# dbdexter-dev/meteor_demod

Measured on AMD Instinct MI355X. Metric: IQ Msamples/s demodulated (whole node), higher is better.
Workload: dtype f32

## Files before the change

meteor_demod_amd/csrc/demod_device.h:

```cpp
#ifndef MDEMOD_DEVICE_H
#define MDEMOD_DEVICE_H

#include <hip/hip_runtime.h>
#include <stdint.h>

#include "pll_flags.h"

#pragma clang fp contract(off)

#define MD_TWO_PI_D 6.283185307179586476925286766559
#define MD_HALF_PI_D 1.5707963267948966192313216916398
#define MD_TWO_PI_F 6.28318548202514648437500f
#define MD_PI_F     3.14159274101257324218750f

struct cf32 { float re, im; };

__device__ __forceinline__ bool md_any(bool p) { return __builtin_amdgcn_ballot_w64(p) != 0ull; }
__device__ __forceinline__ bool md_all(bool p) { return __builtin_amdgcn_ballot_w64(!p) == 0ull; }

template <typename T>
__device__ __forceinline__ T md_lane_select(uint64_t mask, T a, T b)
{
	static_assert(sizeof(T) == 4, "one 32-bit register");
	T r;
// ... 82 lines not shown
{
	return md_fast_sin<CHECKED>((float)((double)fx + MD_HALF_PI_D));
}

__device__ __forceinline__ double
md_sqrt_sumsq(double s)
{
	const double y = __builtin_amdgcn_rsq(s);
	double g = s * y;
	double h = 0.5 * y;
	const double r = __builtin_fma(-h, g, 0.5);
	g = __builtin_fma(g, r, g);
	h = __builtin_fma(h, r, h);
	double d = __builtin_fma(-g, g, s);
	g = __builtin_fma(d, h, g);
	d = __builtin_fma(-g, g, s);
	g = __builtin_fma(d, h, g);
	return __builtin_amdgcn_class(s, 0x260) ? s : g;
}

__device__ __forceinline__ float
md_cabsf_exact(float re, float im)
{
	const double s = (double)re * (double)re + (double)im * (double)im;
	return (float)md_sqrt_sumsq(s);
}

__device__ __forceinline__ float
md_cabsf(float re, float im)
{
	return md_cabsf_exact(re, im);
}

__device__ __forceinline__ float
md_cabsf_short(float re, float im, uint32_t *fallbacks = nullptr)
{
	const double s = (double)re * (double)re + (double)im * (double)im;
	const double y = __builtin_amdgcn_rsq(s);
	const double g = s * y, h = 0.5 * y;
	const double d = __builtin_fma(-g, g, s);
	const double g1 = __builtin_fma(d, h, g);
	const uint64_t gb = __builtin_bit_cast(uint64_t, g1), sb = __builtin_bit_cast(uint64_t, s);
	const uint32_t drop = (uint32_t)gb & 0x1FFFFFFFu;
	const bool near = (uint32_t)(drop - (0x10000000u - 0x1000u)) < 0x2000u;
	const bool odd = (uint32_t)((uint32_t)(sb >> 32) - ((1023u - 200u) << 20)) >= (400u << 20);
	float r = (float)g1;
	if (__builtin_expect(near || odd, 0)) {
		r = (float)md_sqrt_sumsq(s);
		if (fallbacks) *fallbacks += 1;
	}
	return r;
}

__device__ __forceinline__ cf32
md_agc_apply(cf32 x, float gain, float &bias_re, float &bias_im)
{
	const float keep = 1.0f - 0.001f;
	bias_re = bias_re * keep + 0.001f * x.re;
	bias_im = bias_im * keep + 0.001f * x.im;
	x.re = x.re - bias_re;
	x.im = x.im - bias_im;
	x.re = x.re * gain;
	x.im = x.im * gain;
	return x;
}

template <bool SHORT = false>
__device__ __forceinline__ void
md_agc_gain(cf32 scaled, float &gain)
{
	const float mag = SHORT ? md_cabsf_short(scaled.re, scaled.im) : md_cabsf(scaled.re, scaled.im);
	gain = gain + 0.0001f * (190.0f - mag);
	gain = (0.0f > gain) ? 0.0f : gain;
}

template <bool SHORT = false>
__device__ __forceinline__ cf32
md_agc(cf32 x, float &gain, float &bias_re, float &bias_im)
{
	x = md_agc_apply(x, gain, bias_re, bias_im);
	md_agc_gain<SHORT>(x, gain);
	return x;
}

#define MD_TWO_PI_LO (-0x1.777a5cp-23f)

template <bool F32 = false>
__device__ __forceinline__ void
md_nco_advance(float &phase, float freq)
{
	phase = phase + freq;
	if (F32) {
		const float w = (phase - MD_TWO_PI_F) - MD_TWO_PI_LO;
		phase = (phase >= MD_TWO_PI_F) ? w : phase;
	} else if (phase >= MD_TWO_PI_F)
		phase = (float)((double)phase - MD_TWO_PI_D);
}

#define MD_FOUR_PI_F 12.56637096405029296875f
__device__ __forceinline__ float
md_wrap_2pi(float xf)
{
	const bool wraps = !(fabsf(xf) < MD_TWO_PI_F);
	const float once = (xf < 0.0f) ? (xf + MD_TWO_PI_F) + MD_TWO_PI_LO : (xf - MD_TWO_PI_F) - MD_TWO_PI_LO;
	float r = wraps ? once : xf;
	const bool far = !(fabsf(xf) < MD_FOUR_PI_F);
	if (__builtin_expect(md_any(far), 0)) {
		if (far) r = (float)fmod((double)xf, MD_TWO_PI_D);
	}
	return r;
}

__device__ __forceinline__ float
md_tanh_lut(const float *lut, float v)
{
	const float c = __builtin_amdgcn_fmed3f(v, -16.0f, 15.0f);
	return lut[(int)c + 16];
}

__device__ __forceinline__ float
md_tanh_lut_uniform(const float *lut, float v)
{
	float t = (v >= 15.0f) ? 1.0f : -1.0f;
	if (__builtin_expect(md_any(v > -16.0f && v < 15.0f), 0)) t = md_tanh_lut(lut, v);
	return t;
}

__device__ __forceinline__ void
md_tanh_lut_uniform2(const float *lut, float a, float b, float &ta, float &tb)
{
	ta = (a >= 15.0f) ? 1.0f : -1.0f;
	tb = (b >= 15.0f) ? 1.0f : -1.0f;
	if (__builtin_expect(md_any((a > -16.0f && a < 15.0f) || (b > -16.0f && b < 15.0f)), 0)) {
		ta = md_tanh_lut(lut, a);
		tb = md_tanh_lut(lut, b);
	}
}

struct PllState {
	float phase, freq, err;
	int   locked, locked_once, updown;
};

template <bool UNIFORM = false>
__device__ __forceinline__ int
md_pll_update(PllState &p, const float *lut, float alpha, float beta, float fmax,
              float i, float q, int &just_locked_first)
{
	const float e = UNIFORM ? md_tanh_lut_uniform(lut, i) * q - md_tanh_lut_uniform(lut, q) * i
	                        : md_tanh_lut(lut, i) * q - md_tanh_lut(lut, q) * i;

	const float ph = p.phase + alpha * e;
	p.phase = md_wrap_2pi(ph);
	p.freq = p.freq + beta * e;

	const float decayed = p.err * (1.0f - 0.001f);
	p.err = (float)((double)decayed + fabs((double)e) * (double)0.001f);

	const bool lock_now = (p.err < 85.0f) && !p.locked;
	const bool unlock_now = (p.err > 105.0f) && p.locked;
	just_locked_first = (lock_now && !p.locked_once) ? 1 : 0;
	p.locked = lock_now ? 1 : (unlock_now ? 0 : p.locked);
	p.locked_once = lock_now ? 1 : p.locked_once;
	const int changed = (lock_now || unlock_now) ? 1 : 0;
// ... 7 lines not shown
	p.freq = (-fmax > p.freq) ? -fmax : p.freq;
	return changed;
}

struct PllWord { float phase, freq, err; };
template <bool UNIFORM = false, bool EARLY_OUT = false>
__device__ __forceinline__ uint32_t
md_pll_update_packed(PllWord &p, uint32_t &fl, const float *lut, float alpha, float beta, float fmax, float i, float q, uint32_t &first)
{
	float ti, tq;
	if (UNIFORM) md_tanh_lut_uniform2(lut, i, q, ti, tq);
	else { ti = md_tanh_lut(lut, i); tq = md_tanh_lut(lut, q); }
	const float e = ti * q - tq * i;

	const float ph = p.phase + alpha * e;
	p.phase = md_wrap_2pi(ph);
	p.freq = p.freq + beta * e;

	const float decayed = p.err * (1.0f - 0.001f);
	p.err = (float)((double)decayed + fabs((double)e) * (double)0.001f);

	if constexpr (EARLY_OUT) {
		const uint64_t m_below = __builtin_amdgcn_ballot_w64(p.err < 85.0f), m_above = __builtin_amdgcn_ballot_w64(p.err > 105.0f);
		const uint64_t m_locked = __builtin_amdgcn_ballot_w64((fl & 1u) != 0);
		const uint64_t m_lock_event = (m_below & ~m_locked) | (m_above & m_locked);
		const float swept = (float)((double)p.freq + ((fl & 4u) ? 0.000001 : -0.000001));
		p.freq = md_lane_select(m_locked ^ m_lock_event, swept, p.freq);
		const uint64_t m_turn = __builtin_amdgcn_ballot_w64(fabsf(p.freq) >= fmax);
		first = 0;
		uint32_t changed = 0;
		if (__builtin_expect((m_lock_event | m_turn) != 0ull, 0)) {
			const PllFlagStep s = pll_flags_step(fl, md_lane_bit(m_below), md_lane_bit(m_above),
			                                     p.freq >= fmax ? PLL_FREQ_HIGH : (p.freq <= -fmax ? PLL_FREQ_LOW : PLL_FREQ_INSIDE));
			fl = s.fl; first = s.first; changed = s.changed;
		}
		p.freq = md_clamp_sym(p.freq, fmax);
		return changed;
	}

	const uint32_t below = (p.err < 85.0f) ? 1u : 0u, above = (p.err > 105.0f) ? 1u : 0u;
	const uint32_t lock_now = below & (fl ^ 1u);
	const uint32_t unlock_now = above & fl;
	const uint32_t lock2 = lock_now + lock_now;
	first = lock2 ^ (lock2 & fl);
	fl = fl | lock_now | lock2;
	fl = fl ^ (fl & unlock_now);

	if (!(fl & 1u)) p.freq = (float)((double)p.freq + ((fl & 4u) ? 0.000001 : -0.000001));
	fl = (p.freq >= fmax) ? (fl & ~4u) : ((p.freq <= -fmax) ? (fl | 4u) : fl);
	p.freq = md_clamp_sym(p.freq, fmax);
	return lock_now | unlock_now;
}

__device__ __forceinline__ void
md_timing_update(float &t_phase, float &t_freq, float &t_prev,
                 float alpha, float beta, float center, float maxdev, float q)
{
	const float sp = (t_prev < 0.0f) ? -1.0f : 1.0f;
	const float sq = (q < 0.0f) ? -1.0f : 1.0f;
	const float e = sp * q - sq * t_prev;
	t_prev = q;

	float fd = t_freq - center;
	t_phase = (float)((double)t_phase - (MD_TWO_PI_D + (double)(alpha * e)));
	fd = fd - beta * e;
	fd = md_clamp_sym(fd, maxdev);
	t_freq = center + fd;
}

__device__ __forceinline__ int
md_quantise(float v)
{
	const float h = md_clamp_sym(v * 0.5f, 127.0f);
	return (int)h;
}

#endif
```

meteor_demod_amd/csrc/demod_kernel_gat.hip:

```cpp
#include "rotwin_body.h"
#include "hip_host.h"

namespace {

typedef float gpair_t __attribute__((ext_vector_type(2)));
typedef float gquad_t __attribute__((ext_vector_type(4)));
typedef __attribute__((address_space(3))) const gquad_t lds_gquad;
typedef __attribute__((address_space(3))) const float lds_gfloat;

template <int FMT> struct GFmt;
template <> struct GFmt<16> {
	enum { G = 4 };
	__device__ static __forceinline__ gpair_t get(const uint4 &q, int k) { const uint32_t w = (&q.x)[k]; return gpair_t{ (float)(int)(int16_t)(w & 0xFFFFu), (float)((int)w >> 16) }; }
	__device__ static __forceinline__ gpair_t one(uint32_t w) { return gpair_t{ (float)(int)(int16_t)(w & 0xFFFFu), (float)((int)w >> 16) }; }
};
template <> struct GFmt<8> {
	enum { G = 8 };
	__device__ static __forceinline__ gpair_t get(const uint4 &q, int k) { const uint32_t w = (&q.x)[k >> 1] >> (16 * (k & 1)); return gpair_t{ (float)((int)(w & 0xFFu) - 128), (float)((int)((w >> 8) & 0xFFu) - 128) }; }
	__device__ static __forceinline__ gpair_t one(uint16_t w) { return gpair_t{ (float)((int)(w & 0xFFu) - 128), (float)((int)(w >> 8) - 128) }; }
};
template <> struct GFmt<32> {
	enum { G = 2 };
	__device__ static __forceinline__ gpair_t get(const uint4 &q, int k) { return gpair_t{ __uint_as_float((&q.x)[2 * k]), __uint_as_float((&q.x)[2 * k + 1]) }; }
	__device__ static __forceinline__ gpair_t one(float2 w) { return gpair_t{ w.x, w.y }; }
};

template <int KT, int FMT>
struct WinG {
	static constexpr int G = GFmt<FMT>::G, kTaps = KT, kBack = KT - 1, AMAX = G - 1, NS = KT + AMAX, NW = 4 * ((NS + 3) / 4), SLIDE = 4, MAXSL = 1, DEPTH = 1,
	                     BLOCK = MDEMOD_RW_BLOCK, ROTN = 1, RING = 32, REGSLOTS = 0;
	static constexpr bool GATHER = true, SCALAR_SLIDE = false, VCONST = false;
	static constexpr bool LOCK_EARLY_OUT = true;
	static_assert(NS % G == 0 && NS / G <= 36, "whole 16-byte loads, and few enough of them to stay in registers");
	typedef typename RFmt<FMT>::sample_t sample_t;
	__device__ __forceinline__ void setup(uint32_t) {}
	__device__ static __forceinline__ void put_history(const float2 *, bool, int) {}
	__device__ static __forceinline__ void put_init(const RGran<FMT> (&)[1], int) {}
	__device__ static __forceinline__ void put(const RGran<FMT> (&)[1], int) {}
	__device__ static __forceinline__ void fir(uint32_t, int, int, const DemodConsts &, int, float &, float &) {}

	__device__ static __forceinline__ void
	fir_gather(uint32_t ctab_addr, const sample_t *src, const float2 *hist, int v, int n, int bank, const DemodConsts &C, float &re, float &im)
	{
		const int oldest = v - kBack - (KT - 1);
		const int d = oldest & (G - 1);
		const int start = oldest - d;
		const int o = AMAX - d;
		const uint32_t row = ctab_addr + 4u * (uint32_t)(__mul24(bank * 4 + (o & 3), C.ctab_row_stride) + (o & ~3));
		gpair_t acc = { 0.0f, 0.0f };
		if (__builtin_expect(md_all(start >= 0 && start + NS <= n), 1)) {
			uint4 raw[NS / G];
#pragma unroll
			for (int g = 0; g < NS / G; g++) __builtin_memcpy(&raw[g], src + start + G * g, 16);
#pragma unroll
			for (int s4 = 0; s4 < NS / 4; s4++) {
				gquad_t c = { 0.0f, 0.0f, 0.0f, 0.0f };
				c = *(lds_gquad *)(row + 16u * (uint32_t)s4);
				const float cf[4] = { c.x, c.y, c.z, c.w };
#pragma unroll
				for (int k = 0; k < 4; k++) {
					const int slot = 4 * s4 + k;
					const gpair_t smp = GFmt<FMT>::get(raw[slot / G], slot % G);
					const gpair_t p = smp * cf[k];
					acc = acc + p;
				}
			}
			if constexpr (NS % 4 != 0) {
#pragma unroll
				for (int slot = NS / 4 * 4; slot < NS; slot++) {
					const float cf = *(lds_gfloat *)(row + 4u * (uint32_t)slot);
					const gpair_t p = GFmt<FMT>::get(raw[slot / G], slot % G) * cf;
					acc = acc + p;
				}
			}
		} else {
#pragma unroll 1
			for (int k = 0; k < KT; k++) {
				const int idx = oldest + k;
				gpair_t smp;
				if (idx < 0) { const float2 h = hist[kBack + idx]; smp.x = h.x; smp.y = h.y; }
				else smp = GFmt<FMT>::one(src[idx]);
				const float cf = *(lds_gfloat *)(row + 4u * (uint32_t)(d + k));
				const gpair_t p = smp * cf;
				acc = acc + p;
			}
// ... 44 lines not shown
```

meteor_demod_amd/csrc/demod_kernel_rot.hip:

```cpp
#include "rotwin_body.h"
#include "rot_fir_bounds.h"
#include "hip_host.h"
#ifdef ROTWIN_ASM_HEADER
#include ROTWIN_ASM_HEADER
#else
#include "rotwin_asm.h"
#endif

namespace {

static_assert(ROTWIN_NCH * 8 == 80 && ROTWIN_SLIDE == 8, "window = ten chunks of eight, a slide brings one");


__device__ __forceinline__ void
rot_fir(uint32_t row_addr, int rot, int flags, float &re, float &im)
{
	int tmp;
#if ROTWIN_PK == 1 || ROTWIN_PK == 3
	typedef float pair_t __attribute__((ext_vector_type(2)));
	pair_t acc, p0, p1;
	asm volatile(ROTWIN_FIR_ASM
	             : [acc] "=&v"(acc), [p0] "=&v"(p0), [p1] "=&v"(p1), [tmp] "=&s"(tmp)
	             : [addr] "v"(row_addr), [rot] "s"(rot), [flags] "s"(flags)
	             : "vcc", "scc", ROTWIN_COEF_CLOBBERS);
// ... 13 lines not shown
{
	int tmp;
	asm volatile(ROTWIN_PUT_S16_ASM
	             : [tmp] "=&s"(tmp), [rot] "+s"(q), [base] "+s"(base)
	             : [g0] "v"(a.w[0]), [g1] "v"(a.w[1]), [g2] "v"(a.w[2]), [g3] "v"(a.w[3]),
	               [g4] "v"(b.w[0]), [g5] "v"(b.w[1]), [g6] "v"(b.w[2]), [g7] "v"(b.w[3])
	             : "vcc", "scc", "v255", "memory");
}
template <> __device__ __forceinline__ void
rot_put<8>(const RGran<8> &a, const RGran<8> &b, int &q, int &base)
{
	const uint32_t g0 = a.w[0] ^ 0x80808080u, g1 = a.w[1] ^ 0x80808080u, g2 = b.w[0] ^ 0x80808080u, g3 = b.w[1] ^ 0x80808080u;
	int tmp;
	asm volatile(ROTWIN_PUT_U8_ASM
	             : [tmp] "=&s"(tmp), [rot] "+s"(q), [base] "+s"(base)
	             : [g0] "v"(g0), [g1] "v"(g1), [g2] "v"(g2), [g3] "v"(g3)
	             : "vcc", "scc", "v255", "memory");
}
__device__ __forceinline__ void
rot_put_floats(const uint32_t (&f)[16], int &q, int &base)
{
	int tmp;
	asm volatile(ROTWIN_PUT_F32_ASM
	             : [tmp] "=&s"(tmp), [rot] "+s"(q), [base] "+s"(base)
	             : [f0] "v"(f[0]), [f1] "v"(f[1]), [f2] "v"(f[2]), [f3] "v"(f[3]), [f4] "v"(f[4]), [f5] "v"(f[5]), [f6] "v"(f[6]), [f7] "v"(f[7]),
	               [f8] "v"(f[8]), [f9] "v"(f[9]), [f10] "v"(f[10]), [f11] "v"(f[11]), [f12] "v"(f[12]), [f13] "v"(f[13]), [f14] "v"(f[14]), [f15] "v"(f[15])
	             : "vcc", "scc", "v255", "memory");
}
__device__ __forceinline__ void
rot_put_floats(const uint32_t (&f)[16], int q)
{
	int base = 0;
	rot_put_floats(f, q, base);
}
template <> __device__ __forceinline__ void
rot_put<32>(const RGran<32> &a, const RGran<32> &b, int &q, int &base)
{
	uint32_t f[16];
#pragma unroll
	for (int i = 0; i < 8; i++) { f[i] = a.w[i]; f[8 + i] = b.w[i]; }
	rot_put_floats(f, q, base);
}

template <int FMT, int COMPACT = 0, int BLK = MDEMOD_RW_BLOCK, int VC = 0, int RSL = 0>
struct WinF {
	static constexpr int kTaps = 65, kBack = 64, NW = 80, SLIDE = 8, AMAX = NW - kTaps, MAXSL = 1, DEPTH = 1, BLOCK = BLK, ROTN = NW / SLIDE, RING = 32;
	static constexpr bool GATHER = false;
	static constexpr bool SCALAR_SLIDE = true;
	static constexpr bool VCONST = VC != 0;
	static_assert(SLIDE == ROTWIN_SLIDE && ROTN == ROTWIN_NCH, "the slide's assembly counts for itself");
	__device__ __forceinline__ void setup(uint32_t) {}
	static constexpr int REGSLOTS = RSL;
	static constexpr bool LOCK_EARLY_OUT = true;
	__device__ static __forceinline__ void put_history(const float2 *hist, bool valid, int q)
	{
		const uint4 *h4 = reinterpret_cast<const uint4 *>(hist);
		uint32_t f[16];
#pragma unroll
		for (int i = 0; i < 4; i++) {
			uint4 h = h4[i];
			if (!valid) h = make_uint4(0, 0, 0, 0);
			f[4 * i] = h.x; f[4 * i + 1] = h.y; f[4 * i + 2] = h.z; f[4 * i + 3] = h.w;
		}
		rot_put_floats(f, q);
	}
	__device__ static __forceinline__ void put(const RGran<FMT> (&g)[2], int q) { int base = 0; rot_put<FMT>(g[0], g[1], q, base); }
	__device__ static __forceinline__ void put_init(const RGran<FMT> (&g)[2], int q) { put(g, q); }
	__device__ static __forceinline__ void slide(const RGran<FMT> (&g)[2], int &rot, int &base) { rot_put<FMT>(g[0], g[1], rot, base); }
	__device__ static __forceinline__ void fir(uint32_t ctab_addr, int a, int bank, const DemodConsts &C, int rot, float &re, float &im)
	{
		const int o = AMAX - a;
		uint32_t row_addr;
		if (COMPACT) row_addr = rot_mad24((uint32_t)(bank * 4 + (o & 3)), 4u * (uint32_t)C.ctab_row_stride, ctab_addr + 4u * (uint32_t)(o & ~3));
		else row_addr = rot_mad24(rot_mad24((uint32_t)a, (uint32_t)C.interp, (uint32_t)bank), 4u * (uint32_t)C.ctab_row_stride, ctab_addr);
		static_assert(AMAX == 15, "two bits of a / 4");
		const uint64_t ex = __builtin_amdgcn_ballot_w64(true);
		const RotFirQ q = rot_fir_q(ex, __builtin_amdgcn_ballot_w64(a >= 4), __builtin_amdgcn_ballot_w64(a >= 8), __builtin_amdgcn_ballot_w64(a >= 12));
		int q_hi = q.q_hi;
		asm("" : "+s"(q_hi));
		const int flags = rot_fir_flags(q.q_lo, q_hi);
#ifdef ROT_EXP_NOSKIP
		int f0 = __builtin_amdgcn_readfirstlane(flags);
		asm volatile("s_and_b32 %0, %0, 0" : "+s"(f0) : : "scc");
		rot_fir(row_addr, rot, f0, re, im);
#else
		rot_fir(row_addr, rot, flags, re, im);
#endif
	}
};

typedef float pair_t2 __attribute__((ext_vector_type(2)));

template <int NA>
__device__ __forceinline__ void
rot_fir_acc(uint32_t addr, int rot, int last, pair_t2 &acc)
{
	int tmp;
	if constexpr (NA == 10)
		asm volatile(ROTWIN_FIR_ACC_ASM
		             : [acc] "+v"(acc), [tmp] "=&s"(tmp)
		             : [addr] "v"(addr), [rot] "s"(rot), [last] "s"(last)
		             : "vcc", "scc", ROTWIN_COEF_CLOBBERS, ROTWIN_ACC_CLOBBERS);
	else if constexpr (NA == 2)
		asm volatile(ROTWIN_FIR_ACC2_ASM
		             : [acc] "+v"(acc), [tmp] "=&s"(tmp)
		             : [addr] "v"(addr), [rot] "s"(rot), [last] "s"(last)
		             : "vcc", "scc", ROTWIN_COEF_CLOBBERS, ROTWIN_ACC_CLOBBERS);
	else
		asm volatile(ROTWIN_FIR_ACC5_ASM
		             : [acc] "+v"(acc), [tmp] "=&s"(tmp)
		             : [addr] "v"(addr), [rot] "s"(rot), [last] "s"(last)
		             : "vcc", "scc", ROTWIN_COEF_CLOBBERS, ROTWIN_ACC_CLOBBERS);
}
#define ROT_F16_OPERANDS \
	[f0] "v"(f[0]), [f1] "v"(f[1]), [f2] "v"(f[2]), [f3] "v"(f[3]), [f4] "v"(f[4]), [f5] "v"(f[5]), [f6] "v"(f[6]), [f7] "v"(f[7]), \
	[f8] "v"(f[8]), [f9] "v"(f[9]), [f10] "v"(f[10]), [f11] "v"(f[11]), [f12] "v"(f[12]), [f13] "v"(f[13]), [f14] "v"(f[14]), [f15] "v"(f[15])
template <int NA>
__device__ __forceinline__ void
rot_migrate(const uint32_t (&f)[16], int q)
{
	int tmp;
	if constexpr (NA == 10)
		asm volatile(ROTWIN_MIGRATE_ASM : [tmp] "=&s"(tmp) : ROT_F16_OPERANDS, [rot] "s"(q) : "vcc", "scc", "v255", ROTWIN_ACC_CLOBBERS, "memory");
	else if constexpr (NA == 2)
		asm volatile(ROTWIN_MIGRATE2_ASM : [tmp] "=&s"(tmp) : ROT_F16_OPERANDS, [rot] "s"(q) : "vcc", "scc", "v255", ROTWIN_ACC_CLOBBERS, "memory");
	else
		asm volatile(ROTWIN_MIGRATE5_ASM : [tmp] "=&s"(tmp) : ROT_F16_OPERANDS, [rot] "s"(q) : "vcc", "scc", "v255", ROTWIN_ACC_CLOBBERS, "memory");
}
template <int NA>
__device__ __forceinline__ void
rot_put_acc(const uint32_t (&f)[16], int q)
{
	int tmp;
	if constexpr (NA == 10)
		asm volatile(ROTWIN_PUT_ACC_ASM : [tmp] "=&s"(tmp) : ROT_F16_OPERANDS, [rot] "s"(q) : "vcc", "scc", ROTWIN_ACC_CLOBBERS, "memory");
	else if constexpr (NA == 2)
		asm volatile(ROTWIN_PUT_ACC2_ASM : [tmp] "=&s"(tmp) : ROT_F16_OPERANDS, [rot] "s"(q) : "vcc", "scc", ROTWIN_ACC_CLOBBERS, "memory");
	else
		asm volatile(ROTWIN_PUT_ACC5_ASM : [tmp] "=&s"(tmp) : ROT_F16_OPERANDS, [rot] "s"(q) : "vcc", "scc", ROTWIN_ACC_CLOBBERS, "memory");
}

template <int BLK, int NA, int MSL>
struct WinH {
	static constexpr int NR = 10, SLIDE = 8, NW = SLIDE * (NR + NA), kTaps = NA == 10 ? 129 : 65, kBack = kTaps - 1, AMAX = NW - kTaps, MAXSL = MSL, DEPTH = MSL,
	                     BLOCK = BLK, ROTN = NR, RING = 32, REGSLOTS = 0;
	static constexpr bool GATHER = false, SCALAR_SLIDE = false, VCONST = false;
	static constexpr bool LOCK_EARLY_OUT = true;
	static_assert((NA == 10 || NA == 2 || NA == 5) && AMAX == (NA == 5 ? 55 : 31) && kBack % SLIDE == 0, "wide (160 slots, 129 taps), mid (96 slots, 65 taps) or far (120 slots, 65 taps)");
	__device__ __forceinline__ void setup(uint32_t) {}
	__device__ static __forceinline__ void place(const uint32_t (&f)[16], int c)
	{
		if (c < NR) rot_put_floats(f, c);
		else rot_put_acc<NA>(f, c - NR);
	}
	__device__ static __forceinline__ void put_history(const float2 *hist, bool valid, int c)
	{
		const uint4 *h4 = reinterpret_cast<const uint4 *>(hist);
		uint32_t f[16];
#pragma unroll
		for (int i = 0; i < 4; i++) {
			uint4 h = h4[i];
			if (!valid) h = make_uint4(0, 0, 0, 0);
			f[4 * i] = h.x; f[4 * i + 1] = h.y; f[4 * i + 2] = h.z; f[4 * i + 3] = h.w;
		}
		place(f, c);
	}
	__device__ static __forceinline__ void put_init(const RGran<32> (&g)[2], int c)
	{
		uint32_t f[16];
#pragma unroll
		for (int i = 0; i < 8; i++) { f[i] = g[0].w[i]; f[8 + i] = g[1].w[i]; }
		place(f, c);
	}
	__device__ static __forceinline__ void put(const RGran<32> (&g)[2], int q)
	{
		uint32_t f[16];
#pragma unroll
		for (int i = 0; i < 8; i++) { f[i] = g[0].w[i]; f[8 + i] = g[1].w[i]; }
		rot_migrate<NA>(f, q);
	}
	__device__ static __forceinline__ void fir(uint32_t ctab_addr, int a, int bank, const DemodConsts &C, int rot, float &re, float &im)
	{
		const int o = AMAX - a;
		const uint32_t row = ctab_addr + 4u * (uint32_t)(__mul24(bank * 4 + (o & 3), C.ctab_row_stride) + (o & ~3));
		const int flags = (md_all(a >= 8) ? 3 : 0) | ((NA != 10 && md_all(a <= 7)) ? 16 : 0);
		rot_fir(row, rot, __builtin_amdgcn_readfirstlane(flags), re, im);
		if (NA == 10 || md_any(a >= 16)) {
			int last;
			if (NA == 10) last = 6 + (md_any(a >= 8) ? 1 : 0) + (md_any(a >= 16) ? 1 : 0) + (md_any(a >= 24) ? 1 : 0);
			else {
				last = md_any(a >= 24) ? 1 : 0;
				if (NA == 5) last += (md_any(a >= 32) ? 1 : 0) + (md_any(a >= 40) ? 1 : 0) + (md_any(a >= 48) ? 1 : 0);
			}
			pair_t2 acc = { re, im };
			rot_fir_acc<NA>(row + 4u * 80u, NA == 10 ? rot : (NA == 2 ? (rot & 1) : (rot >= 5 ? rot - 5 : rot)), __builtin_amdgcn_readfirstlane(last), acc);
			re = acc.x; im = acc.y;
		}
	}
};

// ... 69 lines not shown
```

meteor_demod_amd/csrc/demod_kernel_rotp.hip:

```cpp
#include "rotwin_body.h"
#include "hip_host.h"
#ifdef ROTPK_ASM_HEADER
#include ROTPK_ASM_HEADER
#else
#include "rotpk_asm.h"
#endif

namespace {

typedef float pair_t __attribute__((ext_vector_type(2)));

template <int GEO> struct GeoP;
#ifndef ROTP_WIDE_DEPTH
#define ROTP_WIDE_DEPTH 1
#endif
#ifndef ROTP_MID_DEPTH
#define ROTP_MID_DEPTH 1
#endif
#ifndef ROTP_FAR_DEPTH
#define ROTP_FAR_DEPTH 2
#endif
template <> struct GeoP<0> { static constexpr int kTaps = 129, NW = MDEMOD_RW_WIDE_NW, MAXSL = 1, DEPTH = ROTP_WIDE_DEPTH, BLOCK = MDEMOD_RW_WIDE_BLOCK; };
template <> struct GeoP<1> { static constexpr int kTaps = 65, NW = MDEMOD_RW_MID_NW, MAXSL = 1, DEPTH = ROTP_MID_DEPTH, BLOCK = MDEMOD_RW_BLOCK; };
#ifndef ROTP_FAR_MAXSL
// ... 6 lines not shown
#if ROTPK_FORM == 0
#define ROTP_FIR_CALL(TEXT, CLOB)                                                                                             \
	float ar = 0.0f, ai = 0.0f;                                                                                               \
	asm volatile(TEXT : [ar] "+v"(ar), [ai] "+v"(ai), [addr] "+v"(addr), [cnt] "+s"(cnt), [tmp] "=&s"(tmp)                    \
	             : [entry] "s"(entry), [sub] "s"(sub) : "vcc", "scc", CLOB);                                                \
	re = ar; im = ai;
#else
#define ROTP_FIR_CALL(TEXT, CLOB)                                                                                             \
	pair_t acc = { 0.0f, 0.0f };                                                                                              \
	asm volatile(TEXT : [acc] "+v"(acc), [addr] "+v"(addr), [cnt] "+s"(cnt), [tmp] "=&s"(tmp)                                 \
	             : [entry] "s"(entry), [sub] "s"(sub) : "vcc", "scc", CLOB);                                                \
	re = acc.x; im = acc.y;
#endif
#define ROTP_ASM(GEO, NAME, FMT)                                                                                              \
	template <> struct AsmP<GEO, FMT> {                                                                                       \
		__device__ static __forceinline__ void fir(uint32_t addr, int entry, int sub, int cnt, float &re, float &im)          \
		{                                                                                                                     \
			int tmp;                                                                                                          \
			ROTP_FIR_CALL(ROTPK_##NAME##_##FMT##_FIR_ASM, ROTPK_##NAME##_##FMT##_CLOBBERS)                                     \
		}                                                                                                                     \
		__device__ static __forceinline__ void put(const uint32_t (&g)[FMT == 16 ? 16 : 8], int q);                           \
	};
ROTP_ASM(0, WIDE, 16) ROTP_ASM(0, WIDE, 8) ROTP_ASM(1, MID, 16) ROTP_ASM(1, MID, 8) ROTP_ASM(2, FAR, 16) ROTP_ASM(2, FAR, 8)

#define ROTP_PUT16(GEO, NAME)                                                                                                 \
	__device__ __forceinline__ void AsmP<GEO, 16>::put(const uint32_t (&g)[16], int q)                                        \
	{                                                                                                                         \
		int tmp;                                                                                                              \
		asm volatile(ROTPK_##NAME##_16_PUT_ASM                                                                                \
		             : [tmp] "=&s"(tmp)                                                                                       \
		             : [g0] "v"(g[0]), [g1] "v"(g[1]), [g2] "v"(g[2]), [g3] "v"(g[3]), [g4] "v"(g[4]), [g5] "v"(g[5]), [g6] "v"(g[6]),  \
		               [g7] "v"(g[7]), [g8] "v"(g[8]), [g9] "v"(g[9]), [g10] "v"(g[10]), [g11] "v"(g[11]), [g12] "v"(g[12]),  \
		               [g13] "v"(g[13]), [g14] "v"(g[14]), [g15] "v"(g[15]), [rot] "s"(q)                                     \
		             : "vcc", "scc", "v255", "memory");                                                                       \
	}
#define ROTP_PUT8(GEO, NAME)                                                                                                  \
	__device__ __forceinline__ void AsmP<GEO, 8>::put(const uint32_t (&g)[8], int q)                                          \
	{                                                                                                                         \
		int tmp;                                                                                                              \
		asm volatile(ROTPK_##NAME##_8_PUT_ASM                                                                                 \
		             : [tmp] "=&s"(tmp)                                                                                       \
		             : [g0] "v"(g[0]), [g1] "v"(g[1]), [g2] "v"(g[2]), [g3] "v"(g[3]), [g4] "v"(g[4]), [g5] "v"(g[5]), [g6] "v"(g[6]),  \
		               [g7] "v"(g[7]), [rot] "s"(q)                                                                           \
		             : "vcc", "scc", "v255", "memory");                                                                       \
	}
ROTP_PUT16(0, WIDE) ROTP_PUT16(1, MID) ROTP_PUT16(2, FAR) ROTP_PUT8(0, WIDE) ROTP_PUT8(1, MID) ROTP_PUT8(2, FAR)

template <int GEO, int FMT>
struct WinP {
	static constexpr int kTaps = GeoP<GEO>::kTaps, kBack = kTaps - 1, NW = GeoP<GEO>::NW, SLIDE = 16, AMAX = NW - kTaps,
	                     MAXSL = GeoP<GEO>::MAXSL, DEPTH = GeoP<GEO>::DEPTH, BLOCK = GeoP<GEO>::BLOCK, NCH = NW / SLIDE, GD = FMT == 16 ? 16 : 8, REGSLOTS = 0, ROTN = NCH, RING = 32;
	static constexpr bool GATHER = false, SCALAR_SLIDE = false, VCONST = false;
	static constexpr bool LOCK_EARLY_OUT = true;
	__device__ __forceinline__ void setup(uint32_t) {}
	static_assert(kBack % SLIDE == 0 && NW % SLIDE == 0, "history and window are whole chunks");

	__device__ static __forceinline__ void put_history(const float2 *hist, bool valid, int q)
	{
		uint32_t g[GD];
#pragma unroll
		for (int k = 0; k < 16; k++) {
			float2 h = hist[k];
			if (!valid) h = make_float2(0.0f, 0.0f);
			if (FMT == 16) {
				g[k] = ((uint32_t)(int)h.x & 0xFFFFu) | ((uint32_t)(int)h.y << 16);
			} else {
				const uint32_t s = (uint32_t)(((int)h.x + 128) & 0xFF) | ((uint32_t)(((int)h.y + 128) & 0xFF) << 8);
				if (k & 1) g[k / 2] |= s << 16; else g[k / 2] = s;
			}
		}
		AsmP<GEO, FMT>::put(g, q);
	}
	__device__ static __forceinline__ void put(const RGran<FMT> (&gr)[4], int q)
	{
		uint32_t g[GD];
#pragma unroll
		for (int i = 0; i < 4; i++)
#pragma unroll
			for (int j = 0; j < GD / 4; j++) g[i * (GD / 4) + j] = gr[i].w[j];
		AsmP<GEO, FMT>::put(g, q);
	}
	__device__ static __forceinline__ void put_init(const RGran<FMT> (&gr)[4], int q) { put(gr, q); }
	__device__ static __forceinline__ void fir(uint32_t ctab_addr, int a, int bank, const DemodConsts &C, int rot, float &re, float &im)
	{
		const int o = AMAX - a;
		uint32_t addr = rot_mad24((uint32_t)(bank * 4 + (o & 3)), 4u * (uint32_t)C.ctab_row_stride, ctab_addr + 4u * (uint32_t)(o & ~3));
		constexpr int QB = AMAX / 4 >= 8 ? 4 : 3;
		static_assert(AMAX / 4 < (1 << QB) && (kTaps - 1) % 4 == 0, "alignments in groups of four");
		int q_lo = 0, q_hi = (1 << QB) - 1;
#pragma unroll
		for (int b = QB - 1; b >= 0; b--) {
			const int t = q_lo + (1 << b);
			q_lo = md_all(a >= 4 * t) ? t : q_lo;
			const int u = q_hi - (1 << b);
			q_hi = md_all(a < 4 * (u + 1)) ? u : q_hi;
		}
		q_lo = __builtin_amdgcn_readfirstlane(q_lo); q_hi = __builtin_amdgcn_readfirstlane(q_hi);
		const int c_lo = q_lo >> 2;
		int chunk = rot + c_lo;
		chunk = chunk >= NCH ? chunk - NCH : chunk;
		const int sub = q_lo & 3;
		constexpr int XS = ROTPK_EXIT / 4;
		const int cnt = (q_hi + (kTaps - 1) / 4) / XS - q_lo / XS;
		AsmP<GEO, FMT>::fir(addr + 64u * (uint32_t)c_lo, __builtin_amdgcn_readfirstlane(chunk), __builtin_amdgcn_readfirstlane(sub), __builtin_amdgcn_readfirstlane(cnt), re, im);
	}
};
// ... 35 lines not shown
```

meteor_demod_amd/csrc/rotwin_body.h:

```cpp
#ifndef MDEMOD_ROTWIN_BODY_H
#define MDEMOD_ROTWIN_BODY_H

#include <hip/hip_runtime.h>
#include <stdint.h>

#include "demod_internal.h"
#include "demod_device.h"
#include "clock_jump.h"
#include "rot_firing_index.h"

#pragma clang fp contract(off)

#ifndef ROT_OQ_SYNC
#define ROT_OQ_SYNC 1
#endif
typedef float rot_sinlut_t;

namespace {

template <int FMT> struct RFmt;
template <> struct RFmt<16> { typedef uint32_t sample_t; enum { GDW = 4 }; };
template <> struct RFmt<8>  { typedef uint16_t sample_t; enum { GDW = 2 }; };
template <> struct RFmt<32> { typedef float2   sample_t; enum { GDW = 8 }; };

// ... 60 lines not shown
		else {
			int k = k_safe;
			for (; k >= 16; k -= 16) p = blind_steps<16>(p, t_freq);
			if (k & 8) p = blind_steps<8>(p, t_freq);
			if (k & 4) p = blind_steps<4>(p, t_freq);
			if (k & 2) p = blind_steps<2>(p, t_freq);
			if (k & 1) p = p + t_freq;
		}
		const float p1 = p + t_freq, p2 = p1 + t_freq, p3 = p2 + t_freq, p4 = p3 + t_freq;
		const bool c1 = p1 >= thr, c2 = p2 >= thr, c3 = p3 >= thr, c4 = p4 >= thr;
		float ph = c3 ? p3 : p4;
		ph = c2 ? p2 : ph;
		ph = c1 ? p1 : ph;
		t_phase = ph;
		if ((KS == 14 || KS == 6) || (KS == 0 && K.tab)) {
			const uint32_t off = (uint32_t)isub + rot_clock_sel(c1, c2, c3);
			const rot_i4 e = *reinterpret_cast<rot_clktab_t>(reinterpret_cast<const __attribute__((address_space(3))) unsigned char *>(K.tab) + off);
			v_cur += e.x;
			isub = e.z;
			bank = e.w;
		} else {
			const int isub_old = isub >> RotIsub<KS>::SHIFT;
			const uint32_t w = (uint32_t)(isub_old + k_safe + 1 + (c1 ? 0 : 1) + (c2 ? 0 : 1) + (c3 ? 0 : 1));
			const uint32_t q = (interp == 1) ? w : __umulhi(w, K.magic);
			const int isub_new = (int)(w - q * (uint32_t)interp);
			v_cur += (int)q + (isub_new > 0 ? 1 : 0) - (isub_old > 0 ? 1 : 0);
			const int fire_sub = (isub_new == 0) ? interp - 1 : isub_new - 1;
			bank = interp - 1 - fire_sub;
			isub = isub_new << RotIsub<KS>::SHIFT;
		}
		fired = c4;
	}
}


template <class W, int FMT, int OQPSK, int KS, int LUT = 0>
__device__ __forceinline__ void
rotwin_demod(const DemodLaunch &L)
{
	typedef typename RFmt<FMT>::sample_t sample_t;
	constexpr int kBack = W::kBack, SLIDE = W::SLIDE, AMAX = W::AMAX, BLOCK = W::BLOCK, NCH = W::NW / W::SLIDE, GPS = W::SLIDE / 4;
	constexpr int NST = GPS * W::DEPTH;
	static_assert(W::DEPTH >= W::MAXSL, "a loop iteration may slide MAXSL times");
	constexpr int ROTN = W::ROTN, RING = W::RING, RGR = RING / 8;
	constexpr bool GATHER = W::GATHER;
	static_assert(RING == 32 || RING == 16, "output ring");
	constexpr int RS = W::REGSLOTS;
#ifndef ROT_PRIO
#define ROT_PRIO 1
#endif
#ifndef ROT_PRIO_LEVEL
#define ROT_PRIO_LEVEL 2
#endif
	constexpr int PRIO = ROT_PRIO;

	extern __shared__ __attribute__((aligned(16))) unsigned char lds[];
	float *ctab = reinterpret_cast<float *>(lds);
	float *lut = ctab + L.ctab_floats;
	enum { S_GAIN, S_BIAS_RE, S_BIAS_IM, S_PHASE, S_FREQ, S_ERR, S_FLAGS, S_TPREV, S_INPHASE, S_EVCALL, S_FIRSTLOCK, S_LASTV, S_COUNT };
	static_assert(S_COUNT == MDEMOD_RW_STATE_SLOTS, "host LDS sizing");
	uint32_t sl_addr = (uint32_t)(uintptr_t)(__attribute__((address_space(3))) unsigned char *)lds
	                   + 4u * (L.ctab_floats + 32u + (threadIdx.x >> 6) * (uint32_t)(S_COUNT * 64) + (threadIdx.x & 63u));
	asm("" : "+v"(sl_addr));
	float *sl = (float *)(__attribute__((address_space(3))) float *)(uintptr_t)sl_addr;
	int *sli = reinterpret_cast<int *>(sl);
	uint4 *stage = reinterpret_cast<uint4 *>(lut + 32 + (BLOCK / 64) * (S_COUNT * 64)) + threadIdx.x;
	const uint32_t ctab_addr = (uint32_t)(uintptr_t)(__attribute__((address_space(3))) unsigned char *)lds;
	W win;
	rot_sinlut_t *sintab = reinterpret_cast<rot_sinlut_t *>(stage - threadIdx.x + BLOCK * RGR);
	if constexpr (LUT) md_sin_lut_fill(sintab, (int)threadIdx.x, BLOCK);
	win.setup(ctab_addr + (uint32_t)(reinterpret_cast<unsigned char *>(stage - threadIdx.x + BLOCK * RGR) - lds) + (LUT ? MDEMOD_SIN_LUT_BYTES : 0));
	rot_i4 *clktab = reinterpret_cast<rot_i4 *>(reinterpret_cast<unsigned char *>(stage - threadIdx.x + BLOCK * RGR) + (LUT ? MDEMOD_SIN_LUT_BYTES : 0));

	const DemodConsts &C = L.c;
	const uint32_t stream = blockIdx.x * blockDim.x + threadIdx.x;
	const bool valid = stream < L.n_streams;

	for (uint32_t i = threadIdx.x; i < L.ctab_floats; i += blockDim.x) ctab[i] = L.ctab[i];
	if (threadIdx.x < 32) lut[threadIdx.x] = L.tanh_lut[threadIdx.x];
	const bool has_clktab = KS != 109 && C.clock_tab != nullptr;
	if (has_clktab)
		for (int i = (int)threadIdx.x; i < 4 * C.interp; i += (int)blockDim.x) {
			rot_i4 e = reinterpret_cast<const rot_i4 *>(C.clock_tab)[i];
			e.z = rot_clock_entry_scaled(e.z);
			clktab[i] = e;
		}

	int n = 0;
	const sample_t *src = nullptr;
	if (valid) {
		n = (int)(L.n_samples_arr ? L.n_samples_arr[stream] : L.n_samples);
		const uint64_t off = L.iq_offset ? L.iq_offset[stream] : (uint64_t)stream * L.iq_stride;
		src = reinterpret_cast<const sample_t *>(L.iq) + off;
	}
	const int v_end = kBack + n;
	const int interp = C.interp;

	float t_phase = 0.0f, t_freq = C.t_center;
	int dual_state = 1;
	float r_gain = 1.0f, r_bias_re = 0.0f, r_bias_im = 0.0f, r_phase = 0.0f, r_freq = 0.0f;
	float r_err = 1000.0f, r_tprev = 0.0f;
	int r_flags = 0, r_lastv = -1;
	auto ld_err = [&]() -> float { return (RS & 1) ? r_err : sl[S_ERR * 64]; };
	auto st_err = [&](float v) { if (RS & 1) r_err = v; else sl[S_ERR * 64] = v; };
	auto ld_tprev = [&]() -> float { return (RS & 2) ? r_tprev : sl[S_TPREV * 64]; };
	auto st_tprev = [&](float v) { if (RS & 2) r_tprev = v; else sl[S_TPREV * 64] = v; };
// ... 98 lines not shown
				if (t_phase >= thr) fired = true;
			}
		}
		if constexpr (GATHER) if (md_all(v_cur == V_DONE)) break;
		ROT_TICK(0);
#ifdef ROT_EXP_TIMING
		n_iter++;
#endif

		bool all_done = false;
		if constexpr (!GATHER)
#pragma unroll
		for (int r = 0; r < W::MAXSL; r++) {
			const int a_now = v_cur - kBack - base;
			if (md_all(a_now >= SLIDE)) {
				if (md_all(v_cur == V_DONE)) { all_done = true; break; }
				RGran<FMT> g[GPS];
#pragma unroll
				for (int i = 0; i < GPS; i++) g[i] = stg[i];
				if constexpr (W::SCALAR_SLIDE) win.slide(g, rot, base);
				else {
					win.put(g, __builtin_amdgcn_readfirstlane(rot));
					rot = __builtin_amdgcn_readfirstlane((rot == ROTN - 1) ? 0 : rot + 1);
					base = __builtin_amdgcn_readfirstlane(base + SLIDE);
				}
#pragma unroll
				for (int i = 0; i + GPS < NST; i++) stg[i] = stg[i + GPS];
				const int m_new = 4 * g_load;
				if (md_all(m_new + SLIDE - 1 < n)) {
#pragma unroll
					for (int i = 0; i < GPS; i++) __builtin_memcpy(&stg[NST - GPS + i], src + m_new + 4 * i, sizeof(RGran<FMT>));
				} else {
#pragma unroll
					for (int i = 0; i < GPS; i++) stg[NST - GPS + i] = rot_fetch<FMT>(src, m_new + 4 * i, n);
				}
				g_load += GPS;
			}
		}
		if (all_done) break;

		ROT_TICK(1);
		const int a = v_cur - kBack - base;
		if (fired && (GATHER || a <= AMAX) && (!(OQPSK && ROT_OQ_SYNC) || dual_state == slot)) {
			fired = false;
			cf32 y;
			if constexpr (GATHER) win.fir_gather(ctab_addr, src, hist_in, v_cur, n, bank, C, y.re, y.im);
			else win.fir(ctab_addr, a, bank, C, W::SCALAR_SLIDE ? rot : __builtin_amdgcn_readfirstlane(rot), y.re, y.im);
			if (PRIO) __builtin_amdgcn_s_setprio(ROT_PRIO_LEVEL);
			ROT_TICK(2);
#ifdef ROT_EXP_TIMING
			n_fir++;
#endif

			y = md_agc<(KS == 14 && !OQPSK && LUT)>(y, r_gain, r_bias_re, r_bias_im);
			uint32_t fl = (uint32_t)ld_flags();
			PllWord pll;
			pll.phase = r_phase; pll.freq = r_freq;
			pll.err = ld_err();

			float sn, cs;
			if constexpr (LUT) {
				sn = md_sin_from_code_lut(sintab, md_turn_code<false>(-pll.phase));
				cs = md_sin_from_code_lut(sintab, md_turn_code<false>((float)((double)(-pll.phase) + MD_HALF_PI_D)));
			} else {
				sn = md_fast_sin<false>(-pll.phase);
				cs = md_fast_cos<false>(-pll.phase);
			}
			bool emit = true;
			float out_re, out_im;
			if (OQPSK) {
				float inphase = sl[S_INPHASE * 64];
				const int rail = ROT_OQ_SYNC ? slot : dual_state;
				if (rail == 1) { inphase = y.re * cs - y.im * sn; emit = false; sl[S_INPHASE * 64] = inphase; }
				out_re = inphase;
				out_im = y.re * sn + y.im * cs;
				dual_state = 3 - rail;
			} else {
				out_re = y.re * cs - y.im * sn;
				out_im = y.re * sn + y.im * cs;
			}
			md_nco_advance<true>(pll.phase, pll.freq);

			if (emit) {
				const bool again = (v_cur == ld_lastv());
				int lastv = v_cur;
				if constexpr ((RS & 8) != 0) asm("" : "+v"(lastv));
				st_lastv(lastv);
				if (__builtin_expect(md_any(again), 0)) {
					if (again) {
						const uint32_t prev = sym_count() - 1u;
						st_symbase(prev & ~(uint32_t)(RING - 1));
						ring_off = rot_ring_off(prev, RING, BLOCK);
					}
				}
				float t_prev = ld_tprev();
				md_timing_update(t_phase, t_freq, t_prev, k_t_alpha, k_t_beta, k_t_center, C.t_maxdev, out_im);
				st_tprev(t_prev);
			}
			rot_clock_fast<KS>(K, OQPSK ? (float)dual_state * MD_PI_F : MD_TWO_PI_F, v_end, v_fast_end, t_phase, t_freq, isub, v_cur, bank, fired,
			                   OQPSK ? (ROT_OQ_SYNC ? 2 - slot : -1) : 0);
#ifdef ROT_EXP_TIMING
			if (!fired) n_slide++;
			if (md_any(!fired)) n_wslow++;
#endif
			if (emit) {
				uint32_t first = 0;
				const uint32_t changed = md_pll_update_packed<false, W::LOCK_EARLY_OUT>(pll,fl, lut, k_pll_alpha, k_pll_beta, C.pll_fmax, out_re, out_im, first);
				if (__builtin_expect(changed != 0, 0)) {
					const uint32_t sym_now = sym_count();
					if (first) sli[S_FIRSTLOCK * 64] = (int)sym_now;
					const int ev_call = sli[S_EVCALL * 64];
					if (ev_call < MDEMOD_MAX_LOCK_EVENTS) {
						mdemod_lock_event ev;
						ev.symbol = L.st.n_symbols[stream] + sym_now; ev.locked = (int)(fl & 1u); ev.pad = 0;
						L.st.events[(size_t)stream * MDEMOD_MAX_LOCK_EVENTS + ev_call] = ev;
					}
					sli[S_EVCALL * 64] = ev_call + 1;
				}
				const uint32_t sym = (uint32_t)(md_quantise(out_re) & 0xFF) | ((uint32_t)(md_quantise(out_im) & 0xFF) << 8);
				*reinterpret_cast<uint16_t *>(reinterpret_cast<unsigned char *>(stage) + ring_off) = (uint16_t)sym;
				ring_off = rot_ring_step(ring_off, RING, BLOCK);
				asm volatile("" : "+v"(r_gain), "+v"(pll.err));
				if (__builtin_expect(ring_off == 0, 0)) {
					const uint32_t sym_call = ld_symbase() + (uint32_t)RING;
					st_symbase(sym_call);
					int8_t *soft_out = L.soft + (size_t)stream * L.soft_stride * 2;
					if (__builtin_expect(sym_call <= L.soft_cap, 1)) {
						int8_t *dst = soft_out + 2 * (size_t)(sym_call - RING);
#pragma unroll
						for (int g4 = 0; g4 < RGR; g4++) {
							const uint4 qv = stage[g4 * BLOCK];
							__builtin_memcpy(dst + 16 * g4, &qv, 16);
							asm volatile("" ::: "memory");
						}
					} else {
						fl |= 8;
						for (uint32_t i = 0; i < (uint32_t)RING && sym_call - RING + i < L.soft_cap; i++)
							*reinterpret_cast<uint16_t *>(soft_out + 2 * (size_t)(sym_call - RING + i)) =
							    reinterpret_cast<const uint16_t *>(stage + (i >> 3) * BLOCK)[i & 7u];
					}
				}
			}
			r_phase = pll.phase; r_freq = pll.freq;
			st_err(pll.err);
			st_flags((int)fl);
			if (PRIO == 1) __builtin_amdgcn_s_setprio(0);
			ROT_TICK(3);
		}
		if (OQPSK && ROT_OQ_SYNC) slot = __builtin_amdgcn_readfirstlane(3 - slot);
	} while (--guard);
#ifdef ROT_EXP_TIMING
	for (int o = 32; o > 0; o >>= 1) n_slide += __shfl_xor(n_slide, o);
	if (blockIdx.x == 100 && threadIdx.x == 0)
		printf("ROT_TIMING iters %u firs %u (lanes left to the stepping loop: %u of the wave's, in %u firings) cycles: clock %llu slide %llu fir %llu scalar %llu latch %llu\n", n_iter, n_fir, n_slide, n_wslow,
		       (unsigned long long)tacc[0], (unsigned long long)tacc[1], (unsigned long long)tacc[2], (unsigned long long)tacc[3], (unsigned long long)tacc[4]);
#endif

	if (guard == 0) st_flags(ld_flags() | 8);

	uint32_t stream_e = stream;
	asm volatile("" : "+v"(stream_e));
	int8_t *soft_e = L.soft + (size_t)stream_e * L.soft_stride * 2;
	int overflow = (ld_flags() >> 3) & 1;

	if (valid) {
		const uint32_t r = rot_ring_count(ring_off, BLOCK), sb = ld_symbase();
		for (uint32_t g = 0; g < (r >> 3); g++) {
			if (sb + 8 * g + 8 <= L.soft_cap) { const uint4 qv = stage[g * BLOCK]; __builtin_memcpy(soft_e + 2 * (size_t)(sb + 8 * g), &qv, 16); }
			else for (uint32_t i = 0; i < 8; i++) {
				if (sb + 8 * g + i < L.soft_cap) *reinterpret_cast<uint16_t *>(soft_e + 2 * (size_t)(sb + 8 * g + i)) = reinterpret_cast<const uint16_t *>(stage + g * BLOCK)[i];
// ... 47 lines not shown
```

Before: 289,000.

## Merge rare-path branches into one wave-uniform slow path in rot kernel

For the register-slot rot window, the per-symbol rare cases (AGC magnitude fallback, repeated-symbol ring rewind, far phase wrap, PLL lock/turn events) are each turned into a ballot mask. They are then combined so the wave tests a single branch instead of several scattered divergent branches. The magnitude fallback and the AGC gain update are deferred until after the PLL update, which moves where they sit in the critical loop. Other window types keep the old path. The combined path adds ballot instructions and can raise register pressure, and its correctness depends on the split helpers matching the original semantics.

Result: faster. 291,900 (median of 6 runs) (+1.0%).

```diff
diff --git a/meteor_demod_amd/csrc/demod_device.h b/meteor_demod_amd/csrc/demod_device.h
--- a/meteor_demod_amd/csrc/demod_device.h
+++ b/meteor_demod_amd/csrc/demod_device.h
@@ -158,6 +158,22 @@
 	return r;
 }
 
+__device__ __forceinline__ float
+md_cabsf_short_try(float re, float im, uint64_t &fallback)
+{
+	const double s = (double)re * (double)re + (double)im * (double)im;
+	const double y = __builtin_amdgcn_rsq(s);
+	const double g = s * y, h = 0.5 * y;
+	const double d = __builtin_fma(-g, g, s);
+	const double g1 = __builtin_fma(d, h, g);
+	const uint64_t gb = __builtin_bit_cast(uint64_t, g1), sb = __builtin_bit_cast(uint64_t, s);
+	const uint32_t drop = (uint32_t)gb & 0x1FFFFFFFu;
+	const bool near = (uint32_t)(drop - (0x10000000u - 0x1000u)) < 0x2000u;
+	const bool odd = (uint32_t)((uint32_t)(sb >> 32) - ((1023u - 200u) << 20)) >= (400u << 20);
+	fallback = __builtin_amdgcn_ballot_w64(near) | __builtin_amdgcn_ballot_w64(odd);
+	return (float)g1;
+}
+
 __device__ __forceinline__ cf32
 md_agc_apply(cf32 x, float gain, float &bias_re, float &bias_im)
 {
@@ -180,6 +196,13 @@
 	gain = (0.0f > gain) ? 0.0f : gain;
 }
 
+__device__ __forceinline__ float
+md_agc_gain_step(float gain, float mag)
+{
+	gain = gain + 0.0001f * (190.0f - mag);
+	return (0.0f > gain) ? 0.0f : gain;
+}
+
 template <bool SHORT = false>
 __device__ __forceinline__ cf32
 md_agc(cf32 x, float &gain, float &bias_re, float &bias_im)
@@ -216,6 +239,16 @@
 	}
 	return r;
 }
+
+__device__ __forceinline__ float
+md_wrap_2pi_near(float xf, bool &far)
+{
+	const bool wraps = !(fabsf(xf) < MD_TWO_PI_F);
+	const float once = (xf < 0.0f) ? (xf + MD_TWO_PI_F) + MD_TWO_PI_LO : (xf - MD_TWO_PI_F) - MD_TWO_PI_LO;
+	far = !(fabsf(xf) < MD_FOUR_PI_F);
+	return wraps ? once : xf;
+}
+__device__ __forceinline__ float md_wrap_2pi_far(float xf) { return (float)fmod((double)xf, MD_TWO_PI_D); }
 
 __device__ __forceinline__ float
 md_tanh_lut(const float *lut, float v)
@@ -329,6 +362,37 @@
 	return lock_now | unlock_now;
 }
 
+__device__ __forceinline__ uint64_t
+md_pll_update_common(PllWord &p, uint32_t fl, const float *lut, float alpha, float beta, float fmax, float i, float q, float &ph, bool &far)
+{
+	const float ti = md_tanh_lut(lut, i), tq = md_tanh_lut(lut, q);
+	const float e = ti * q - tq * i;
+
+	ph = p.phase + alpha * e;
+	p.phase = md_wrap_2pi_near(ph, far);
+	p.freq = p.freq + beta * e;
+
+	const float decayed = p.err * (1.0f - 0.001f);
+	p.err = (float)((double)decayed + fabs((double)e) * (double)0.001f);
+
+	const uint64_t m_below = __builtin_amdgcn_ballot_w64(p.err < 85.0f), m_above = __builtin_amdgcn_ballot_w64(p.err > 105.0f);
+	const uint64_t m_locked = __builtin_amdgcn_ballot_w64((fl & 1u) != 0);
+	const uint64_t m_lock_event = (m_below & ~m_locked) | (m_above & m_locked);
+	const float swept = (float)((double)p.freq + ((fl & 4u) ? 0.000001 : -0.000001));
+	p.freq = md_lane_select(m_locked ^ m_lock_event, swept, p.freq);
+	const uint64_t m_turn = __builtin_amdgcn_ballot_w64(fabsf(p.freq) >= fmax);
+	return m_lock_event | m_turn;
+}
+
+__device__ __forceinline__ uint32_t
+md_pll_update_rare(const PllWord &p, uint32_t &fl, float fmax, uint32_t &first)
+{
+	const PllFlagStep s = pll_flags_step(fl, p.err < 85.0f ? 1u : 0u, p.err > 105.0f ? 1u : 0u,
+	                                     p.freq >= fmax ? PLL_FREQ_HIGH : (p.freq <= -fmax ? PLL_FREQ_LOW : PLL_FREQ_INSIDE));
+	fl = s.fl; first = s.first;
+	return s.changed;
+}
+
 __device__ __forceinline__ void
 md_timing_update(float &t_phase, float &t_freq, float &t_prev,
                  float alpha, float beta, float center, float maxdev, float q)
diff --git a/meteor_demod_amd/csrc/demod_kernel_gat.hip b/meteor_demod_amd/csrc/demod_kernel_gat.hip
--- a/meteor_demod_amd/csrc/demod_kernel_gat.hip
+++ b/meteor_demod_amd/csrc/demod_kernel_gat.hip
@@ -31,6 +31,7 @@
 	                     BLOCK = MDEMOD_RW_BLOCK, ROTN = 1, RING = 32, REGSLOTS = 0;
 	static constexpr bool GATHER = true, SCALAR_SLIDE = false, VCONST = false;
 	static constexpr bool LOCK_EARLY_OUT = true;
+	static constexpr bool RARE_ONE_BRANCH = false;
 	static_assert(NS % G == 0 && NS / G <= 36, "whole 16-byte loads, and few enough of them to stay in registers");
 	typedef typename RFmt<FMT>::sample_t sample_t;
 	__device__ __forceinline__ void setup(uint32_t) {}
diff --git a/meteor_demod_amd/csrc/demod_kernel_rot.hip b/meteor_demod_amd/csrc/demod_kernel_rot.hip
--- a/meteor_demod_amd/csrc/demod_kernel_rot.hip
+++ b/meteor_demod_amd/csrc/demod_kernel_rot.hip
@@ -89,6 +89,7 @@
 	__device__ __forceinline__ void setup(uint32_t) {}
 	static constexpr int REGSLOTS = RSL;
 	static constexpr bool LOCK_EARLY_OUT = true;
+	static constexpr bool RARE_ONE_BRANCH = true;
 	__device__ static __forceinline__ void put_history(const float2 *hist, bool valid, int q)
 	{
 		const uint4 *h4 = reinterpret_cast<const uint4 *>(hist);
@@ -183,6 +184,7 @@
 	                     BLOCK = BLK, ROTN = NR, RING = 32, REGSLOTS = 0;
 	static constexpr bool GATHER = false, SCALAR_SLIDE = false, VCONST = false;
 	static constexpr bool LOCK_EARLY_OUT = true;
+	static constexpr bool RARE_ONE_BRANCH = false;
 	static_assert((NA == 10 || NA == 2 || NA == 5) && AMAX == (NA == 5 ? 55 : 31) && kBack % SLIDE == 0, "wide (160 slots, 129 taps), mid (96 slots, 65 taps) or far (120 slots, 65 taps)");
 	__device__ __forceinline__ void setup(uint32_t) {}
 	__device__ static __forceinline__ void place(const uint32_t (&f)[16], int c)
diff --git a/meteor_demod_amd/csrc/demod_kernel_rotp.hip b/meteor_demod_amd/csrc/demod_kernel_rotp.hip
--- a/meteor_demod_amd/csrc/demod_kernel_rotp.hip
+++ b/meteor_demod_amd/csrc/demod_kernel_rotp.hip
@@ -82,6 +82,7 @@
 	                     MAXSL = GeoP<GEO>::MAXSL, DEPTH = GeoP<GEO>::DEPTH, BLOCK = GeoP<GEO>::BLOCK, NCH = NW / SLIDE, GD = FMT == 16 ? 16 : 8, REGSLOTS = 0, ROTN = NCH, RING = 32;
 	static constexpr bool GATHER = false, SCALAR_SLIDE = false, VCONST = false;
 	static constexpr bool LOCK_EARLY_OUT = true;
+	static constexpr bool RARE_ONE_BRANCH = false;
 	__device__ __forceinline__ void setup(uint32_t) {}
 	static_assert(kBack % SLIDE == 0 && NW % SLIDE == 0, "history and window are whole chunks");
 
diff --git a/meteor_demod_amd/csrc/rotwin_body.h b/meteor_demod_amd/csrc/rotwin_body.h
--- a/meteor_demod_amd/csrc/rotwin_body.h
+++ b/meteor_demod_amd/csrc/rotwin_body.h
@@ -136,6 +136,7 @@
 #ifndef ROT_PRIO_LEVEL
 #define ROT_PRIO_LEVEL 2
 #endif
+	constexpr bool RARE = W::RARE_ONE_BRANCH;
 	constexpr int PRIO = ROT_PRIO;
 
 	extern __shared__ __attribute__((aligned(16))) unsigned char lds[];
@@ -340,7 +341,13 @@
 			n_fir++;
 #endif
 
-			y = md_agc<(KS == 14 && !OQPSK && LUT)>(y, r_gain, r_bias_re, r_bias_im);
+			constexpr bool SHORT_ABS = KS == 14 && !OQPSK && LUT;
+			float mag = 0.0f;
+			uint64_t m_abs = 0;
+			if constexpr (RARE && SHORT_ABS) {
+				y = md_agc_apply(y, r_gain, r_bias_re, r_bias_im);
+				mag = md_cabsf_short_try(y.re, y.im, m_abs);
+			} else y = md_agc<SHORT_ABS>(y, r_gain, r_bias_re, r_bias_im);
 			uint32_t fl = (uint32_t)ld_flags();
 			PllWord pll;
 			pll.phase = r_phase; pll.freq = r_freq;
@@ -369,18 +376,22 @@
 			}
 			md_nco_advance<true>(pll.phase, pll.freq);
 
+			uint64_t m_again = 0;
+			auto ring_back = [&]() {
+				const uint32_t prev = sym_count() - 1u;
+				st_symbase(prev & ~(uint32_t)(RING - 1));
+				ring_off = rot_ring_off(prev, RING, BLOCK);
+			};
 			if (emit) {
 				const bool again = (v_cur == ld_lastv());
+				if constexpr (RARE) { m_again = __builtin_amdgcn_ballot_w64(again); asm volatile("" : "+s"(m_again)); }
 				int lastv = v_cur;
 				if constexpr ((RS & 8) != 0) asm("" : "+v"(lastv));
 				st_lastv(lastv);
-				if (__builtin_expect(md_any(again), 0)) {
-					if (again) {
-						const uint32_t prev = sym_count() - 1u;
-						st_symbase(prev & ~(uint32_t)(RING - 1));
-						ring_off = rot_ring_off(prev, RING, BLOCK);
+				if constexpr (!RARE)
+					if (__builtin_expect(md_any(again), 0)) {
+						if (again) ring_back();
 					}
-				}
 				float t_prev = ld_tprev();
 				md_timing_update(t_phase, t_freq, t_prev, k_t_alpha, k_t_beta, k_t_center, C.t_maxdev, out_im);
 				st_tprev(t_prev);
@@ -393,17 +404,35 @@
 #endif
 			if (emit) {
 				uint32_t first = 0;
-				const uint32_t changed = md_pll_update_packed<false, W::LOCK_EARLY_OUT>(pll,fl, lut, k_pll_alpha, k_pll_beta, C.pll_fmax, out_re, out_im, first);
-				if (__builtin_expect(changed != 0, 0)) {
+				auto lock_event = [&](uint32_t fl_now) {
 					const uint32_t sym_now = sym_count();
 					if (first) sli[S_FIRSTLOCK * 64] = (int)sym_now;
 					const int ev_call = sli[S_EVCALL * 64];
 					if (ev_call < MDEMOD_MAX_LOCK_EVENTS) {
 						mdemod_lock_event ev;
-						ev.symbol = L.st.n_symbols[stream] + sym_now; ev.locked = (int)(fl & 1u); ev.pad = 0;
+						ev.symbol = L.st.n_symbols[stream] + sym_now; ev.locked = (int)(fl_now & 1u); ev.pad = 0;
 						L.st.events[(size_t)stream * MDEMOD_MAX_LOCK_EVENTS + ev_call] = ev;
 					}
 					sli[S_EVCALL * 64] = ev_call + 1;
+				};
+				if constexpr (RARE) {
+					float ph;
+					bool far;
+					const uint64_t m_pll = md_pll_update_common(pll, fl, lut, k_pll_alpha, k_pll_beta, C.pll_fmax, out_re, out_im, ph, far);
+					const uint64_t rare = m_pll | __builtin_amdgcn_ballot_w64(far) | m_again | m_abs;
+					if (__builtin_expect(rare != 0ull, 0)) {
+						if (md_lane_bit(m_abs)) mag = md_cabsf_exact(y.re, y.im);
+						if (md_lane_bit(m_again)) ring_back();
+						if (far) pll.phase = md_wrap_2pi_far(ph);
+						uint32_t fl_new = fl;
+						if (md_pll_update_rare(pll, fl_new, C.pll_fmax, first)) lock_event(fl_new);
+						asm volatile("v_mov_b32 %0, %1" : "+v"(fl) : "v"(fl_new));
+					}
+					pll.freq = md_clamp_sym(pll.freq, C.pll_fmax);
+					if constexpr (SHORT_ABS) r_gain = md_agc_gain_step(r_gain, mag);
+				} else {
+					const uint32_t changed = md_pll_update_packed<false, W::LOCK_EARLY_OUT>(pll,fl, lut, k_pll_alpha, k_pll_beta, C.pll_fmax, out_re, out_im, first);
+					if (__builtin_expect(changed != 0, 0)) lock_event(fl);
 				}
 				const uint32_t sym = (uint32_t)(md_quantise(out_re) & 0xFF) | ((uint32_t)(md_quantise(out_im) & 0xFF) << 8);
 				*reinterpret_cast<uint16_t *>(reinterpret_cast<unsigned char *>(stage) + ring_off) = (uint16_t)sym;
```
